# nikhilTkur/Multigrid_Nikhil_C-

Measured on AMD Instinct MI355X. Metric: fine_grid_stencil_updates_per_sec, higher is better.
Workload: dtype f64

## Files before the change

multigrid_nikhil_c-_amd/csrc/mgx_kernels.hpp:

```cpp
#pragma once

#include <hip/hip_runtime.h>
#include "mgx_geom.hpp"
#include <stdint.h>
#include <type_traits>

namespace mgx {

template <int B, int E, typename F> __device__ __forceinline__ void static_for(F&& f)
{
    if constexpr (B < E) {
        f(std::integral_constant<int, B>{});
        static_for<B + 1, E>(f);
    }
}

constexpr int kWave = 64;
constexpr int kBlock = 256;
constexpr int kWavesPerBlock = kBlock / kWave;
constexpr int kOutLanes = kWave - 2;

template <typename T> struct VecOf;
template <> struct VecOf<double> { using type = double2; static constexpr int W = 2; };
template <> struct VecOf<float>  { using type = float4;  static constexpr int W = 4; };
// ... 638 lines not shown
    double a0 = 0.0, a1 = 0.0, a2 = 0.0, a3 = 0.0;
    int i = threadIdx.x;
    for (; i + 3 * kReduceThreads < n; i += 4 * kReduceThreads) {
        a0 += partial[i];
        a1 += partial[i + kReduceThreads];
        a2 += partial[i + 2 * kReduceThreads];
        a3 += partial[i + 3 * kReduceThreads];
    }
    for (; i < n; i += kReduceThreads) a0 += partial[i];
    double acc = (a0 + a1) + (a2 + a3);
    for (int off = 32; off > 0; off >>= 1) acc += __shfl_down(acc, off, kWave);
    if ((threadIdx.x & 63) == 0) wsum[threadIdx.x >> 6] = acc;
    __syncthreads();
    if (threadIdx.x == 0) {
        double s = 0.0;
        for (int w = 0; w < kReduceThreads / kWave; ++w) s += wsum[w];
        out[0] = s;
    }
}

template <typename T> struct Trip { T l, c, r; };

template <typename T, bool FUSED>
__global__ void __launch_bounds__(kBlock)
k_restrict(const T* __restrict__ vin, const T* __restrict__ rhs, T* __restrict__ coarse, T* __restrict__ coarse_zero,
           int N, long pitch, long cpitch, int crow_lo, int crow_hi, int fine_row_off,
           int R, int strips, int chunks, T wgt)
{
    using V = typename VecOf<T>::type;
    constexpr int W = VecOf<T>::W;
    constexpr int CW = W / 2;
    const Tile t = wave_tile(strips, chunks);
    if (!t.active) return;
    const Cols c = lane_cols<W>(t.strip, N, pitch);
    const int I0 = crow_lo + t.chunk * R;
    const int I1 = min(I0 + R, crow_hi);
    const T* pv = vin + c.col;
    const T* pb = rhs + c.col;
    const long ccol = c.col / 2;
    const int NC = N / 2;

    auto row_plain = [&](int y) -> V { V o = vload<V>(pb + (long)y * pitch, c.ld); mask_cols(o, c.col, N); return o; };

    V up, cur, dn;
    int yf = 2 * I0 + fine_row_off - 1;
    if (FUSED) {
        up = vload<V>(pv + (long)(yf - 1) * pitch, c.ld);
        cur = vload<V>(pv + (long)yf * pitch, c.ld);
    }
    auto next_field = [&](int y) -> V {
        if (FUSED) {
            dn = vload<V>(pv + (long)(y + 1) * pitch, c.ld);
            const V bb = vload<V>(pb + (long)y * pitch, c.ld);
            V o = residual_vec(up, cur, dn, bb);
            mask_cols(o, c.col, N);
            up = cur; cur = dn;
            return o;
        } else {
            return row_plain(y);
        }
    };
    auto trips = [&](const V& f, Trip<T>* tr) {
        const T l = from_left(last(f));
        if constexpr (W == 2) { tr[0] = {l, f.x, f.y}; }
        else { tr[0] = {l, f.x, f.y}; tr[1] = {f.y, f.z, f.w}; }
    };

    Trip<T> top[CW], mid[CW], bot[CW];
    { const V f = next_field(yf); trips(f, top); }
    for (int I = I0; I < I1; ++I) {
        const int y = 2 * I + fine_row_off;
        { const V f = next_field(y); trips(f, mid); }
        { const V f = next_field(y + 1); trips(f, bot); }
        T o[CW];
#pragma unroll
        for (int k = 0; k < CW; ++k) {
            T corners = top[k].l + top[k].r; corners = corners + bot[k].l; corners = corners + bot[k].r;
            T edges = mid[k].l + mid[k].r; edges = edges + top[k].c; edges = edges + bot[k].c;
            o[k] = wgt * ((corners + (T)2 * edges) + (T)4 * mid[k].c);
            if (ccol + k == 0 || ccol + k >= NC) o[k] = (T)0;
        }
        if (c.st) {
            T* pc = coarse + (long)I * cpitch + ccol;
            if constexpr (CW == 1) { pc[0] = o[0]; }
            else { *reinterpret_cast<float2*>(pc) = make_float2((float)o[0], (float)o[1]); }
            if (coarse_zero) {
                T* pz = coarse_zero + (long)I * cpitch + ccol;
                if constexpr (CW == 1) { pz[0] = (T)0; }
                else { *reinterpret_cast<float2*>(pz) = make_float2(0.f, 0.f); }
            }
        }
#pragma unroll
        for (int k = 0; k < CW; ++k) top[k] = bot[k];
    }
}

template <typename T, bool ADD>
__global__ void __launch_bounds__(kBlock)
k_prolong(T* __restrict__ v, const T* __restrict__ coarse, int N, long pitch, long cpitch,
          int row_lo, int row_hi, int fine_row_off, int R, int strips, int chunks)
{
    using V = typename VecOf<T>::type;
    constexpr int W = VecOf<T>::W;
    constexpr int CW = W / 2;
    const Tile t = wave_tile(strips, chunks);
    if (!t.active) return;
    const Cols c = lane_cols<W>(t.strip, N, pitch);
    const int r0 = row_lo + t.chunk * R;
    const int r1 = min(r0 + R, row_hi);
    T* pv = v + c.col;
    const long ccol = c.col / 2;
    const bool cld = c.ld && (ccol + CW < cpitch);

    auto crow = [&](int I, T* e) {
        const T* p = coarse + (long)I * cpitch + ccol;
#pragma unroll
        for (int k = 0; k <= CW; ++k) e[k] = cld ? p[k] : (T)0;
    };
    for (int r = r0; r < r1; ++r) {
        const int y = r - fine_row_off;
        const int I = y >> 1;
        T a[CW + 1], b2[CW + 1];
        crow(I, a);
        V add;
        T o[W];
        if ((y & 1) == 0) {
#pragma unroll
            for (int k = 0; k < CW; ++k) { o[2 * k] = a[k]; o[2 * k + 1] = (T)0.5 * (a[k] + a[k + 1]); }
        } else {
            crow(I + 1, b2);
#pragma unroll
            for (int k = 0; k < CW; ++k) {
                o[2 * k] = (T)0.5 * (a[k] + b2[k]);
                o[2 * k + 1] = (T)0.25 * (((a[k] + b2[k]) + a[k + 1]) + b2[k + 1]);
            }
        }
        if constexpr (W == 2) add = make_double2(o[0], o[1]);
        else add = make_float4(o[0], o[1], o[2], o[3]);
        mask_cols(add, c.col, N);
        if (ADD) {
            const V old = vload<V>(pv + (long)r * pitch, c.st);
            if constexpr (W == 2) { add.x = old.x + add.x; add.y = old.y + add.y; }
            else { add.x = old.x + add.x; add.y = old.y + add.y; add.z = old.z + add.z; add.w = old.w + add.w; }
        }
        vstore<V>(pv + (long)r * pitch, add, c.st);
    }
}

template <int K, int POST> constexpr int cycle_halo_cols() { return K + (POST == 1 ? 2 : (POST == 2 ? 1 : 0)); }
template <int K, int POST, int W> constexpr int cycle_out_lanes() { return kWave - 2 * ((cycle_halo_cols<K, POST>() + W - 1) / W); }

template <typename T, int CW> struct CycleState {
    T ct[CW], tc[CW], em[CW], mc[CW];
    double acc;
};

struct CycleWin {
    int row_first, row_last;
    int crow_first, crow_last;
    int emit_lo, emit_hi;
};

struct CycleArgs {
    long cpitch; int NC;
    int r0, r1, y_end;
    bool zero_in;
    CycleWin win;
};

template <typename T, int CW> struct PreFetch { T a[CW + 1], b[CW + 1]; };

template <typename T, bool EDGE>
__device__ __forceinline__ void
coarse_loads(PreFetch<T, VecOf<T>::W / 2>& pe, int y, const T* __restrict__ coarse_e, long cpitch, long ccol, int N, bool cld,
             const CycleWin& win, const FastOut& fo)
{
    constexpr int CW = VecOf<T>::W / 2;
    const int I = y >> 1;
    if constexpr (!EDGE) {
        const int Ia = min(max(I, win.crow_first), win.crow_last), Ib = min(max(I + 1, win.crow_first), win.crow_last);
        const unsigned srow_a = (unsigned)(Ia - fo.crb) * fo.cpitch_bytes, srow_b = (unsigned)(Ib - fo.crb) * fo.cpitch_bytes;
#pragma unroll
        for (int k = 0; k <= CW; ++k) pe.a[k] = bload1_s((T*)nullptr, fo.ce, fo.clane_off + (unsigned)(k * sizeof(T)), srow_a);
#pragma unroll
        for (int k = 0; k <= CW; ++k) pe.b[k] = bload1_s((T*)nullptr, fo.ce, fo.clane_off + (unsigned)(k * sizeof(T)), srow_b);
    } else {
        const bool cl = cld && y > 0 && y < N && I >= win.crow_first && I + (y & 1) <= win.crow_last;
        const bool cl2 = cl && (y & 1);
        const unsigned at = (unsigned)(I - fo.crb) * fo.cpitch_bytes + fo.clane_off;
#pragma unroll
        for (int k = 0; k <= CW; ++k) pe.a[k] = bload1((T*)nullptr, fo.ce, cl ? at + (unsigned)(k * sizeof(T)) : kOobOffset);
#pragma unroll
        for (int k = 0; k <= CW; ++k) pe.b[k] = bload1((T*)nullptr, fo.ce, cl2 ? at + fo.cpitch_bytes + (unsigned)(k * sizeof(T)) : kOobOffset);
    }
}

template <typename T, bool EDGE, bool ZIN = false>
__device__ __forceinline__ void
cycle_loads(typename VecOf<T>::type& in, typename VecOf<T>::type& bn, int y,
            const T* __restrict__ pv, const T* __restrict__ pb, long pitch, int N, int y_end, bool ld, bool zero_in,
            const CycleWin& win, const FastOut& fo)
{
    using V = typename VecOf<T>::type;
    if constexpr (!EDGE) {
        const int yi = min(y, win.row_last), yb = max(min(y - 1, win.row_last), win.row_first);
        if constexpr (ZIN) in = vzero((V*)nullptr);
        else in = bload_s((V*)nullptr, fo.in, fo.lane_off, (unsigned)(yi - fo.rb) * fo.pitch_bytes);
        bn = bload_s((V*)nullptr, fo.rhs, fo.lane_off, (unsigned)(yb - fo.rb) * fo.pitch_bytes);
    } else {
        const bool in_ok = !zero_in && y >= win.row_first && y <= win.row_last && y < y_end;
        const bool b_ok = (y - 1) > 0 && (y - 1) < N && (y - 1) >= win.row_first && (y - 1) <= win.row_last && y <= y_end;
        in = bload((V*)nullptr, fo.in, (ld && in_ok) ? (unsigned)(y - fo.rb) * fo.pitch_bytes + fo.lane_off : kOobOffset);
        bn = bload((V*)nullptr, fo.rhs, (ld && b_ok) ? (unsigned)(y - 1 - fo.rb) * fo.pitch_bytes + fo.lane_off : kOobOffset);
    }
}

constexpr int kBRing = 12;
template <typename T, int K, int POST, int SM> constexpr bool cycle_b_in_lds() { return (sizeof(T) == 8 && K >= 8) || (sizeof(T) == 4 && K >= 10); }
#ifndef MGX_SKEW
#define MGX_SKEW 0
#endif
#ifndef MGX_RING_AHEAD
#define MGX_RING_AHEAD 1
#endif
#ifndef MGX_PRIO_ALT
#define MGX_PRIO_ALT 0
#endif
template <typename T, int K, int PRE, int POST, int SM, int AR> constexpr int cycle_skew()
{
    if (sizeof(T) == 8 && K == 10 && PRE == 1 && POST == 0 && SM == 0 && AR == 0) return 0;
    if (sizeof(T) == 4 && K == 10 && PRE == 0 && POST == 1 && SM == 0) return 0;
    return (MGX_SKEW != 0 && cycle_b_in_lds<T, K, POST, SM>()) ? K / 2 : 0;
}
constexpr int kRawLds = 6;
#ifndef MGX_RAWQ
#define MGX_RAWQ 1
#endif
template <typename T, int K, int PRE, int POST, int SM, int AR> constexpr bool cycle_rawq();
template <typename T> struct LdsVec;
template <> struct LdsVec<double> { typedef double v __attribute__((ext_vector_type(2))); };
template <> struct LdsVec<float> { typedef float v __attribute__((ext_vector_type(4))); };
template <typename T> using lds_vec_ptr = __attribute__((address_space(3))) typename LdsVec<T>::v*;
__device__ __forceinline__ void ring_put(lds_vec_ptr<double> r, int slot, const double2& v)
{
    LdsVec<double>::v t = {v.x, v.y};
    r[slot * kWave] = t;
}
__device__ __forceinline__ double2 ring_get(lds_vec_ptr<double> r, int slot)
{
    const LdsVec<double>::v t = r[slot * kWave];
    return make_double2(t.x, t.y);
}
__device__ __forceinline__ void ring_put(lds_vec_ptr<float> r, int slot, const float4& v)
{
    LdsVec<float>::v t = {v.x, v.y, v.z, v.w};
    r[slot * kWave] = t;
}
__device__ __forceinline__ float4 ring_get(lds_vec_ptr<float> r, int slot)
{
    const LdsVec<float>::v t = r[slot * kWave];
    return make_float4(t.x, t.y, t.z, t.w);
}
constexpr int ring_slot(int m) { return ((m % kBRing) + kBRing) % kBRing; }
template <typename T, int K, int PRE, int POST, int SM, int AR> constexpr bool cycle_rawq()
{
    if (MGX_RAWQ == 0) return false;
    if (PRE != 0 || sizeof(T) != 8) return false;
    if (POST == 2 && AR == 0 && K == 10) return false;
    return cycle_b_in_lds<T, K, POST, SM>() && SM == 0 && POST != 0 && K > kRawLds && cycle_skew<T, K, PRE, POST, SM, AR>() == 0;
}
#ifndef MGX_PFD_DEEP
#define MGX_PFD_DEEP 0
#endif
template <bool BL, int POST, bool EDGE = false> constexpr int cycle_pfd()
{
    if (BL && !EDGE && MGX_PFD_DEEP > 0) return MGX_PFD_DEEP;
    return (BL && (POST == 1 || EDGE)) ? 2 : kPrefetch;
}
constexpr int kPrefetchMax = MGX_PFD_DEEP > kPrefetch ? MGX_PFD_DEEP : kPrefetch;
template <typename T, bool BL, bool EDGE, int POST> constexpr int cycle_cpfd() { return (BL && !(EDGE && POST == 0)) ? cycle_pfd<BL, POST, EDGE>() : 1; }

template <typename T, int K, int PRE, int POST, int SM, bool EDGE, int RP, bool BL, bool ZIN, int AR>
__device__ __forceinline__ void
cycle_step(typename VecOf<T>::type (&lev)[K + 1][3], typename VecOf<T>::type (&bw)[BL ? 1 : K + 1], lds_vec_ptr<T> ring,
           lds_vec_ptr<T> ring2, typename VecOf<T>::type (&rawq)[cycle_rawq<T, K, PRE, POST, SM, AR>() ? kBRing : 1],
           typename VecOf<T>::type (&nin)[kPfStages], typename VecOf<T>::type (&nbn)[kPfStages], PreFetch<T, VecOf<T>::W / 2>& pe,
           CycleState<T, VecOf<T>::W / 2>& cs, int y,
           const T* __restrict__ pv, const T* __restrict__ pb, T* __restrict__ po,
           const T* __restrict__ coarse_e, T* __restrict__ coarse_b, T* __restrict__ coarse_zero, T wgt,
           long pitch, long col, long ccol, int N, const CycleArgs& ca, bool ld, bool cld, bool st, T c0, T c1,
           const FastOut& fo)
{
    using V = typename VecOf<T>::type;
    constexpr int W = VecOf<T>::W;
    constexpr int CW = W / 2;
    constexpr int P = RP % 3;
    constexpr int S_OLD = (P + 1) % 3, S_MID = (P + 2) % 3, S_NEW = P;
    constexpr int bnd_lo = 0;
    const int bnd_hi = N;
    const int r0 = ca.r0, r1 = ca.r1;

    if constexpr (EDGE) __builtin_amdgcn_sched_barrier(0);
    V in = nin[0];
    const V bn = nbn[0];
#pragma unroll
    for (int q = 0; q + 1 < kPfStages; ++q) { nin[q] = nin[q + 1]; nbn[q] = nbn[q + 1]; }
    cycle_loads<T, EDGE, ZIN>(nin[kPfStages - 1], nbn[kPfStages - 1], y + cycle_pfd<BL, POST, EDGE>(), pv, pb, pitch, N, ca.y_end, ld, ca.zero_in, ca.win, fo);
    const ColMask cm = col_mask(col, N);
    if (PRE) {
        T a[CW + 1], b2[CW + 1], o[W];
#pragma unroll
        for (int k = 0; k <= CW; ++k) { a[k] = pe.a[k]; b2[k] = pe.b[k]; }
        coarse_loads<T, EDGE>(pe, y + cycle_cpfd<T, BL, EDGE, POST>(), coarse_e, ca.cpitch, ccol, N, cld, ca.win, fo);
        {
            const bool even = (y & 1) == 0;
#pragma unroll
            for (int k = 0; k < CW; ++k) {
                const T ab = a[k] + b2[k];
                const T ev1 = (T)0.5 * (a[k] + a[k + 1]);
                const T od0 = (T)0.5 * ab;
                const T od1 = (T)0.25 * ((ab + a[k + 1]) + b2[k + 1]);
                o[2 * k] = even ? a[k] : od0;
                o[2 * k + 1] = even ? ev1 : od1;
            }
        }
        V add;
        if constexpr (W == 2) add = make_double2(o[0], o[1]);
        else add = make_float4(o[0], o[1], o[2], o[3]);
        if constexpr (EDGE) mask_sel(add, cm, false);
        if constexpr (W == 2) { in.x = in.x + add.x; in.y = in.y + add.y; }
        else { in.x = in.x + add.x; in.y = in.y + add.y; in.z = in.z + add.z; in.w = in.w + add.w; }
    }
    constexpr bool RAWQ = cycle_rawq<T, K, PRE, POST, SM, AR>();
    constexpr bool PREMUL = (SM == 0 && POST == 0) || RAWQ;
    V b0;
    if constexpr (PREMUL) b0 = vscale(c1, bn);
    else b0 = bn;
    if constexpr (BL) {
        asm volatile("" : "+v"(ring));
        ring_put(ring, ring_slot(RP), b0);
        if constexpr (RAWQ) {
            asm volatile("" : "+v"(ring2));
            rawq[ring_slot(RP)] = ring_get(ring2, RP % kRawLds);
            ring_put(ring2, RP % kRawLds, bn);
        }
    } else {
#pragma unroll
        for (int j = K; j > 0; --j) bw[j] = bw[j - 1];
        bw[0] = b0;
    }
    constexpr int kRingAhead = MGX_RING_AHEAD;
    constexpr int SK = cycle_skew<T, K, PRE, POST, SM, AR>();
    constexpr int SKD = SK > 0 ? 1 : 0;
    constexpr int MLAST = ((POST && !RAWQ) ? K : K - 1) + SKD;
    V rq[BL ? K + 2 : 1];
    auto bwin = [&](auto jc) -> V {
        constexpr int j = decltype(jc)::value;
        if constexpr (j == 0) return b0;
        else if constexpr (BL) return rq[j];
        else return bw[j];
    };
    V dying = lev[SK][S_NEW];
    lev[0][S_NEW] = in;
    auto level = [&](auto jc, auto bc) {
        constexpr int j = decltype(jc)::value;
        constexpr bool inB = decltype(bc)::value;
        const int row = y - j - (inB ? 1 : 0);
        const V cb = bwin(std::integral_constant<int, j - 1 + (inB ? 1 : 0)>{});
        const V& lo = (inB && j == SK + 1) ? dying : lev[j - 1][S_OLD];
        const V& mi = (inB && j == SK + 1) ? lev[j - 1][S_OLD] : lev[j - 1][S_MID];
        const V& hi = (inB && j == SK + 1) ? lev[j - 1][S_MID] : lev[j - 1][S_NEW];
        V o;
        if constexpr (PREMUL) o = jacobi_vec_pre<AR>(lo, mi, hi, cb, c0, c1);
        else o = level_op<T, SM, AR>(j, lo, mi, hi, cb, c0, c1, row + (int)(col & 1));
        if constexpr (EDGE) {
            const int rw = opaque_s(row);
            mask_sel(o, cm, !(rw > bnd_lo && rw < bnd_hi));
        }
        if constexpr (j == K) {
            const unsigned at = (unsigned)(row - fo.rb) * fo.pitch_bytes + fo.lane_off;
            bstore(o, fo.out, (st && row >= r0 && row < r1) ? at : kOobOffset);
        }
        if (j < K || POST) lev[j][S_NEW] = o;
    };
    if constexpr (SK == 0) {
        if constexpr (BL) {
            static_for<1, (kRingAhead < MLAST ? kRingAhead : MLAST) + 1>([&](auto mc) {
                constexpr int m = decltype(mc)::value;
                rq[m] = ring_get(ring, ring_slot(RP - m));
            });
        }
        static_for<1, K + 1>([&](auto jc) {
            constexpr int j = decltype(jc)::value;
            if constexpr (BL && j + kRingAhead <= MLAST) {
                rq[j + kRingAhead] = ring_get(ring, ring_slot(RP - (j + kRingAhead)));
                __builtin_amdgcn_sched_barrier(0);
            }
            level(jc, std::false_type{});
        });
    } else {
        constexpr int NB = K - SK;
        constexpr int NP = SK > NB ? SK : NB;
        rq[SK + 1] = ring_get(ring, ring_slot(RP - (SK + 1)));
        static_for<1, NP + 1>([&](auto ic) {
            constexpr int i = decltype(ic)::value;
            if constexpr (i + 1 <= SK) rq[i] = ring_get(ring, ring_slot(RP - i));
            if constexpr (i + 1 <= NB) rq[SK + i + 1] = ring_get(ring, ring_slot(RP - (SK + i + 1)));
            if constexpr (POST != 0 && i == NP) rq[K + 1] = ring_get(ring, ring_slot(RP - (K + 1)));
            __builtin_amdgcn_sched_barrier(0);
            if constexpr (i <= SK) level(std::integral_constant<int, i>{}, std::false_type{});
            if constexpr (i <= NB) level(std::integral_constant<int, SK + i>{}, std::true_type{});
        });
    }
    if (POST) {
        const int rho = y - K - 1 - SKD;
        V rawb;
        if constexpr (RAWQ) rawb = rawq[ring_slot(RP - (K - kRawLds))];
        else rawb = bwin(std::integral_constant<int, K + SKD>{});
        V res = residual_vec(lev[K][S_OLD], lev[K][S_MID], lev[K][S_NEW], rawb);
        if constexpr (EDGE) {
            const int rw = opaque_s(rho);
            mask_sel(res, cm, !(rw > bnd_lo && rw < bnd_hi));
        }
        if (POST == 2) {
            double r2;
            if constexpr (W == 2) r2 = (double)res.x * (double)res.x + (double)res.y * (double)res.y;
            else r2 = ((double)res.x * (double)res.x + (double)res.y * (double)res.y) +
                      ((double)res.z * (double)res.z + (double)res.w * (double)res.w);
            cs.acc += (st && rho >= r0 && rho < r1) ? r2 : 0.0;
        } else {
            T cl[CW], cc[CW], cr[CW];
            const T l = from_left(last(res));
            if constexpr (W == 2) { cl[0] = l; cc[0] = res.x; cr[0] = res.y; }
            else { cl[0] = l; cc[0] = res.x; cr[0] = res.y; cl[1] = res.y; cc[1] = res.z; cr[1] = res.w; }
            const bool odd = (rho & 1) != 0;
            const int I = (rho - 1) >> 1;
            const bool emit = odd && (2 * I >= r0) && (2 * I < r1) && I >= ca.win.emit_lo && I < ca.win.emit_hi;
            T o[CW];
#pragma unroll
            for (int k = 0; k < CW; ++k) {
                T corners = cs.ct[k] + cl[k]; corners = corners + cr[k];
                const T edges = cs.em[k] + cc[k];
                o[k] = wgt * ((corners + (T)2 * edges) + (T)4 * cs.mc[k]);
                if constexpr (EDGE) o[k] = (ccol + k == 0 || ccol + k >= ca.NC) ? (T)0 : o[k];
            }
            {
                const unsigned at = (st && emit) ? ((unsigned)(I - fo.crb) * fo.cpitch_bytes + fo.clane_off) : kOobOffset;
                if constexpr (CW == 1) { bstore8(o[0], fo.cb, at); bstore8((T)0, fo.cz, at); }
                else { bstore8(make_float2((float)o[0], (float)o[1]), fo.cb, at); bstore8(make_float2(0.f, 0.f), fo.cz, at); }
            }
#pragma unroll
            for (int k = 0; k < CW; ++k) {
                const T lr = cl[k] + cr[k];
                const T em = lr + cs.tc[k];
                cs.em[k] = odd ? cs.em[k] : em;
                cs.mc[k] = odd ? cs.mc[k] : cc[k];
                cs.ct[k] = odd ? lr : cs.ct[k];
                cs.tc[k] = odd ? cc[k] : cs.tc[k];
            }
        }
    }
}

template <typename T, int K, int PRE, int POST, int SM, bool EDGE, bool ZIN, int AR>
__device__ __forceinline__ double
cycle_body(const T* __restrict__ pv, const T* __restrict__ pb, T* __restrict__ po,
           const T* __restrict__ coarse_e, T* __restrict__ coarse_b, T* __restrict__ coarse_zero, T wgt,
           long pitch, long cpitch, long col, int N, int r0, int r1, bool ld, bool st, T c0, T c1, bool zero_in,
           const CycleWin& win, lds_vec_ptr<T> ring, lds_vec_ptr<T> ring2, const FastOut& fo)
{
    constexpr bool BL = cycle_b_in_lds<T, K, POST, SM>();
    constexpr bool RAWQ = cycle_rawq<T, K, PRE, POST, SM, AR>();
    using V = typename VecOf<T>::type;
    constexpr int W = VecOf<T>::W;
    constexpr int CW = W / 2;
    constexpr int ETOP = POST ? 1 : 0;
    constexpr int EBOT = POST == 1 ? 2 : (POST == 2 ? 1 : 0);
    const V Z = vzero((V*)nullptr);
    const long ccol = col / 2;
    const bool cld = ld && (ccol + CW < cpitch);
    V lev[K + 1][3];
    V bw[BL ? 1 : K + 1];
#pragma unroll
    for (int j = 0; j <= K; ++j) { lev[j][0] = Z; lev[j][1] = Z; lev[j][2] = Z; }
#pragma unroll
    for (int j = 0; j < (BL ? 1 : K + 1); ++j) bw[j] = Z;
    if constexpr (BL) {
#pragma unroll
        for (int q = 0; q < kBRing; ++q) ring_put(ring, q, Z);
    }
    V rawq[RAWQ ? kBRing : 1];
#pragma unroll
    for (int q = 0; q < (RAWQ ? kBRing : 1); ++q) rawq[q] = Z;
    if constexpr (RAWQ) {
#pragma unroll
        for (int q = 0; q < kRawLds; ++q) ring_put(ring2, q, Z);
    }
    CycleState<T, CW> cs;
    cs.acc = 0.0;
#pragma unroll
    for (int k = 0; k < CW; ++k) cs.ct[k] = cs.tc[k] = cs.em[k] = cs.mc[k] = (T)0;
    CycleArgs ca;
    ca.cpitch = cpitch; ca.NC = N / 2; ca.r0 = r0; ca.r1 = r1; ca.zero_in = zero_in; ca.win = win;
    const int y0 = r0 - K - ETOP;
    ca.y_end = r1 + K + EBOT + (cycle_skew<T, K, PRE, POST, SM, AR>() > 0 ? 1 : 0);
    constexpr int kRound = BL ? kBRing : trip_steps<T>();
    const int steps = (ca.y_end - y0 + kRound - 1) / kRound * kRound;
    constexpr int PFD = cycle_pfd<BL, POST, EDGE>();
    V nin[PFD][kPfStages], nbn[PFD][kPfStages];
    constexpr int CPFD = cycle_cpfd<T, BL, EDGE, POST>();
    PreFetch<T, CW> pe[CPFD];
#pragma unroll
    for (int q = 0; q < CPFD; ++q) {
#pragma unroll
        for (int k = 0; k <= CW; ++k) { pe[q].a[k] = (T)0; pe[q].b[k] = (T)0; }
    }
#pragma unroll
    for (int q = 0; q < PFD; ++q)
        cycle_loads<T, EDGE, ZIN>(nin[q][0], nbn[q][0], y0 + q, pv, pb, pitch, N, ca.y_end, ld, ca.zero_in, ca.win, fo);
    if (PRE) {
#pragma unroll
        for (int q = 0; q < CPFD; ++q) coarse_loads<T, EDGE>(pe[q], y0 + q, coarse_e, cpitch, ccol, N, cld, ca.win, fo);
    }
#define MGX_CSTEP(RP, Y) cycle_step<T, K, PRE, POST, SM, EDGE, RP, BL, ZIN, AR>(lev, bw, ring, ring2, rawq, nin[(RP) % PFD], nbn[(RP) % PFD], pe[(RP) % CPFD], cs, Y, pv, pb, po, coarse_e, coarse_b, coarse_zero, wgt, pitch, col, ccol, N, ca, ld, cld, st, c0, c1, fo)
    if constexpr (BL) {
#define MGX_CTRIP(Y) do { MGX_CSTEP(0, Y); MGX_CSTEP(1, Y + 1); MGX_CSTEP(2, Y + 2); MGX_CSTEP(3, Y + 3); MGX_CSTEP(4, Y + 4); \
                          MGX_CSTEP(5, Y + 5); MGX_CSTEP(6, Y + 6); MGX_CSTEP(7, Y + 7); MGX_CSTEP(8, Y + 8); MGX_CSTEP(9, Y + 9); \
                          MGX_CSTEP(10, Y + 10); MGX_CSTEP(11, Y + 11); } while (0)
#if MGX_PRIO_ALT
        unsigned hw_id;
        asm volatile("s_getreg_b32 %0, hwreg(HW_REG_HW_ID)" : "=s"(hw_id));
        int turn = (int)(hw_id & 1u);
        for (int y = y0; y < y0 + steps; y += kBRing) {
            if (turn & 1) __builtin_amdgcn_s_setprio(1); else __builtin_amdgcn_s_setprio(0);
            turn ^= 1;
            MGX_CTRIP(y);
        }
        __builtin_amdgcn_s_setprio(0);
#else
        for (int y = y0; y < y0 + steps; y += kBRing) MGX_CTRIP(y);
#endif
#undef MGX_CTRIP
    } else if constexpr (trip_steps<T>() == 12) {
        for (int y = y0; y < y0 + steps; y += 12) {
            MGX_CSTEP(0, y); MGX_CSTEP(1, y + 1); MGX_CSTEP(2, y + 2);
            MGX_CSTEP(3, y + 3); MGX_CSTEP(4, y + 4); MGX_CSTEP(5, y + 5);
            MGX_CSTEP(6, y + 6); MGX_CSTEP(7, y + 7); MGX_CSTEP(8, y + 8);
            MGX_CSTEP(9, y + 9); MGX_CSTEP(10, y + 10); MGX_CSTEP(11, y + 11);
        }
    } else {
        for (int y = y0; y < y0 + steps; y += 3) {
            MGX_CSTEP(0, y); MGX_CSTEP(1, y + 1); MGX_CSTEP(2, y + 2);
        }
    }
#undef MGX_CSTEP
    return cs.acc;
}

template <typename T, int K, int PRE, int POST, int SM, int AR> constexpr int cycle_waves()
{
    return cycle_b_in_lds<T, K, POST, SM>() ? 2 : 1;
}
template <typename T, int K, int PRE, int POST, int SM = 0, int AR = 0>
__global__ void __launch_bounds__(kBlock, (cycle_waves<T, K, PRE, POST, SM, AR>()))
k_jacobi_cycle(const T* __restrict__ vin, const T* __restrict__ rhs, T* __restrict__ vout,
               const T* __restrict__ coarse_e,
               T* __restrict__ coarse_b, T* __restrict__ coarse_zero, T wgt,
               double* __restrict__ partial,
               int N, long pitch, long cpitch, int row_lo, int row_hi, int R, int strips, int chunks, int Re, int chunks_e,
               int row_last0, int Rl, int RB, int n_tall, int n_short, int Rf, T c0, T c1, int zero_in, CycleWin win)
{
    constexpr int W = VecOf<T>::W;
    constexpr int XC = cycle_halo_cols<K, POST>();
    constexpr int HL = (XC + W - 1) / W;
    constexpr int OUT = kWave - 2 * HL;
    constexpr int ETOP = POST ? 1 : 0;
    constexpr int EBOT = POST == 1 ? 2 : (POST == 2 ? 1 : 0);
    __shared__ double wsum[kWavesPerBlock];
    constexpr bool BL = cycle_b_in_lds<T, K, POST, SM>();
    __shared__ typename LdsVec<T>::v bring[BL ? kWavesPerBlock * kBRing * kWave : 1];
    constexpr bool RAWQ = cycle_rawq<T, K, PRE, POST, SM, AR>();
    __shared__ typename LdsVec<T>::v braw[RAWQ ? kWavesPerBlock * kRawLds * kWave : 1];
    const CTile t = cycle_tile(strips, chunks, chunks_e, R, Re, row_lo, row_hi, row_last0, Rl, RB, n_tall, n_short, Rf);
    double acc = 0.0;
#ifdef MGX_WAVE_TRACE
    const long long trace_t0 = wall_clock64();
#endif
    if (t.active) {
        const int lane = threadIdx.x & 63;
        const int wv = __builtin_amdgcn_readfirstlane(threadIdx.x >> 6);
        lds_vec_ptr<T> ring = (lds_vec_ptr<T>)&bring[BL ? (wv * kBRing * kWave + lane) : 0];
        lds_vec_ptr<T> ring2 = (lds_vec_ptr<T>)&braw[RAWQ ? (wv * kRawLds * kWave + lane) : 0];
        const int vx0 = t.strip * OUT - HL;
        const int vx = vx0 + lane;
        const long col = (long)vx * W;
        const bool ld = (vx >= 0) && (col + W <= pitch);
        const bool st = (lane >= HL) && (lane < kWave - HL) && (vx < N / W);
        const int r0 = t.r0, r1 = t.r1;
        constexpr int kRound = BL ? kBRing : trip_steps<T>();
        const int y_first = r0 - K - ETOP - 1;
        constexpr int SKD = cycle_skew<T, K, PRE, POST, SM, AR>() > 0 ? 1 : 0;
        const int y_lastp = (r0 - K - ETOP) + ((r1 + K + EBOT + SKD) - (r0 - K - ETOP) + kRound - 1) / kRound * kRound + kPrefetchMax;
        const int y0c = r0 - K - ETOP, y1c = r1 + K + EBOT - 1;
        bool interior = (vx0 >= 1) && ((long)(vx0 + kWave + 1) * W < N) &&
                        (y0c > 0) && (y1c < N) && (y0c >= win.row_first) && (y1c <= win.row_last);
        if (PRE) interior = interior && (y0c >> 1) >= win.crow_first && ((y1c + 1) >> 1) <= win.crow_last;
        interior = interior && !(PRE != 0 && zero_in);
        FastOut fo;
        fo.rb = max(y_first, win.row_first);
        fo.crb = max(y_first >> 1, win.crow_first);
        fo.pitch_bytes = (unsigned)(pitch * (long)sizeof(T));
        fo.cpitch_bytes = (unsigned)(cpitch * (long)sizeof(T));
        const unsigned f_bytes = rsrc_bytes(fo.rb, win.row_last, fo.pitch_bytes);
        const unsigned c_bytes = rsrc_bytes(fo.crb, win.crow_last, fo.cpitch_bytes);
        const long f_at = (long)fo.rb * pitch, c_at = (long)fo.crb * cpitch;
        fo.out = make_rsrc(vout + f_at, f_bytes);
        fo.in = make_rsrc(vin + f_at, f_bytes);
        fo.rhs = make_rsrc(rhs + f_at, f_bytes);
        fo.ce = make_rsrc(PRE ? coarse_e + c_at : nullptr, (PRE && coarse_e) ? c_bytes : 0u);
        fo.cb = make_rsrc((POST == 1 && coarse_b) ? coarse_b + c_at : nullptr, (POST == 1 && coarse_b) ? c_bytes : 0u);
        fo.cz = make_rsrc((POST == 1 && coarse_zero) ? coarse_zero + c_at : nullptr, (POST == 1 && coarse_zero) ? c_bytes : 0u);
        fo.lane_off = (unsigned)(col * (long)sizeof(T));
        fo.clane_off = (unsigned)((col / 2) * (long)sizeof(T));
        if (interior) {
            if (PRE == 0 && zero_in)
                acc = cycle_body<T, K, PRE, POST, SM, false, PRE == 0, AR>(vin + col, rhs + col, vout + col, coarse_e, coarse_b, coarse_zero, wgt,
                                                                      pitch, cpitch, col, N, r0, r1, true, st, c0, c1, true, win, ring, ring2, fo);
            else
                acc = cycle_body<T, K, PRE, POST, SM, false, false, AR>(vin + col, rhs + col, vout + col, coarse_e, coarse_b, coarse_zero, wgt,
                                                                    pitch, cpitch, col, N, r0, r1, true, st, c0, c1, false, win, ring, ring2, fo);
        } else {
            acc = cycle_body<T, K, PRE, POST, SM, true, false, AR>(vin + col, rhs + col, vout + col, coarse_e, coarse_b, coarse_zero, wgt,
                                                        pitch, cpitch, col, N, r0, r1, ld, st, c0, c1, zero_in != 0, win, ring, ring2, fo);
        }
    }
#ifdef MGX_WAVE_TRACE
    if ((threadIdx.x & 63) == 0) {
        const int w = blockIdx.x * kWavesPerBlock + (threadIdx.x >> 6);
        if (w < (1 << 16)) {
            unsigned hw, xcc;
            asm volatile("s_getreg_b32 %0, hwreg(HW_REG_HW_ID)" : "=s"(hw));
            asm volatile("s_getreg_b32 %0, hwreg(HW_REG_XCC_ID)" : "=s"(xcc));
            g_wave_trace[w] = WaveTrace{trace_t0, wall_clock64(), t.active ? t.strip : -1, t.r0, t.r1,
                                        (int)((hw & 0xFFF0FFFFu) | ((xcc & 0xFu) << 16))};
        }
        if (w == 0) g_wave_trace_n = gridDim.x * kWavesPerBlock;
    }
#endif
    if (POST == 2) {
        for (int off = 32; off > 0; off >>= 1) acc += __shfl_down(acc, off, kWave);
        if ((threadIdx.x & 63) == 0) wsum[threadIdx.x >> 6] = acc;
        __syncthreads();
        if (threadIdx.x == 0) {
            double sum = 0.0;
            for (int w = 0; w < kWavesPerBlock; ++w) sum += wsum[w];
            partial[blockIdx.x] = sum;
        }
    }
}

constexpr int kTileBand = 14;
constexpr int kTileSY = kWavesPerBlock * kTileBand;
constexpr int kTileSX = kWave;

template <int POST> constexpr int tile_extra() { return POST == 1 ? 2 : (POST == 2 ? 1 : 0); }

template <typename T, int SM, int PRE, int POST, int AR = 0>
__global__ void __launch_bounds__(kBlock)
k_tile_smooth(const T* __restrict__ vin, const T* __restrict__ rhs, T* __restrict__ vout,
              const T* __restrict__ coarse_e, T* __restrict__ coarse_b, T* __restrict__ coarse_zero, T wgt,
              double* __restrict__ partial, int N, long pitch, long cpitch, int levels, T c0, T c1,
              int tiles_x, int zero_in, int row_lo, int row_hi, CycleWin win)
{
    constexpr int RW = kTileBand;
    __shared__ T edge[2][kWavesPerBlock][2][kWave];
    __shared__ double wsum[kWavesPerBlock];
    const int He = levels + tile_extra<POST>();
    const int TH = kTileSY - 2 * He, TW = kTileSX - 2 * He;
    const int lane = threadIdx.x & 63;
    const int wv = __builtin_amdgcn_readfirstlane(threadIdx.x >> 6);
    const int ty = blockIdx.x / tiles_x, tx = blockIdx.x - ty * tiles_x;
    const int y0 = wv * RW;
    const int gy0 = row_lo + ty * TH - He + y0;
    const int gx = 1 + tx * TW - He + lane;
    const bool colunk = gx > 0 && gx < N;
    const int NC = N / 2;

    T u[RW], b[RW];
    unsigned rowmask = 0;
#pragma unroll
    for (int i = 0; i < RW; ++i) {
        const int gy = gy0 + i;
        const bool rowok = gy > 0 && gy < N && gy >= win.row_first && gy <= win.row_last;
        if (rowok) rowmask |= 1u << i;
        const bool unk = colunk && rowok;
        const long at = (long)gy * pitch + gx;
        u[i] = (unk && !zero_in) ? vin[at] : (T)0;
        b[i] = unk ? rhs[at] : (T)0;
    }
    if (PRE) {
        const bool codd = (gx & 1) != 0;
#pragma unroll
        for (int i = 0; i < RW; ++i) {
            const int gy = gy0 + i;
            const bool rodd = (gy & 1) != 0;
            const bool unk = colunk && ((rowmask >> i) & 1u) && (gy >> 1) >= win.crow_first && (gy >> 1) + (rodd ? 1 : 0) <= win.crow_last;
            const T* e = coarse_e + (long)(gy >> 1) * cpitch + (gx >> 1);
            const T a00 = unk ? e[0] : (T)0;
            const T a01 = (unk && codd) ? e[1] : (T)0;
            const T a10 = (unk && rodd) ? e[cpitch] : (T)0;
            const T a11 = (unk && rodd && codd) ? e[cpitch + 1] : (T)0;
            const T ev = codd ? (T)0.5 * (a00 + a01) : a00;
            const T od = codd ? (T)0.25 * (((a00 + a10) + a01) + a11) : (T)0.5 * (a00 + a10);
            const T add = rodd ? od : ev;
            u[i] = unk ? u[i] + add : u[i];
        }
    }

    int buf = 0;
    auto halo_rows = [&](const T (&a)[RW], T& up, T& dn) {
        edge[buf][wv][0][lane] = a[0];
        edge[buf][wv][1][lane] = a[RW - 1];
        __syncthreads();
        up = wv > 0 ? edge[buf][wv - 1][1][lane] : (T)0;
        dn = wv < kWavesPerBlock - 1 ? edge[buf][wv + 1][0][lane] : (T)0;
        buf ^= 1;
    };
    for (int j = 1; j <= levels; ++j) {
        T up, dn;
        halo_rows(u, up, dn);
        const bool colact = colunk && lane >= j && lane < kTileSX - j;
        const int ilo = max(j - y0, 0), ihi = min(kTileSY - j - y0, RW);
        const unsigned act = ihi > ilo ? (rowmask & (((1u << (ihi - ilo)) - 1u) << ilo)) : 0u;
        T prev = up;
#pragma unroll
        for (int i = 0; i < RW; ++i) {
            const T cur = u[i];
            const T below = (i == RW - 1) ? dn : u[i + 1];
            const T l = from_left(cur), r = from_right(cur);
            const bool rowact = (act >> i) & 1u;
            if (SM == 0) {
                const T o = jac_pt<AR>(c0, cur, c1 * b[i], c1, nbr(prev, l, r, below));
                u[i] = (colact && rowact) ? o : cur;
            } else {
                const T o = (T)0.25 * (b[i] + nbr(prev, l, r, below));
                u[i] = (colact && rowact && ((gy0 + i + gx) & 1) == ((j - 1) & 1)) ? o : cur;
            }
            prev = cur;
        }
    }

    const bool colout = lane >= He && lane < He + TW && gx < N;
#pragma unroll
    for (int i = 0; i < RW; ++i) {
        const int y = y0 + i, gy = gy0 + i;
        if (y >= He && y < He + TH && gy < N && gy >= row_lo && gy < row_hi && colout) vout[(long)gy * pitch + gx] = u[i];
    }

// ... 389 lines not shown
```

Measured before the change: 1077 billion.

## Specialize fused cycle steps on compile-time row parity to halve coarse loads

```diff
diff --git a/multigrid_nikhil_c-_amd/csrc/mgx_kernels.hpp b/multigrid_nikhil_c-_amd/csrc/mgx_kernels.hpp
--- a/multigrid_nikhil_c-_amd/csrc/mgx_kernels.hpp
+++ b/multigrid_nikhil_c-_amd/csrc/mgx_kernels.hpp
@@ -814,6 +814,7 @@
 
 template <typename T, int CW> struct CycleState {
     T ct[CW], tc[CW], em[CW], mc[CW];
+    T ea[CW + 1];
     double acc;
 };
 
@@ -854,6 +855,24 @@
         for (int k = 0; k <= CW; ++k) pe.a[k] = bload1((T*)nullptr, fo.ce, cl ? at + (unsigned)(k * sizeof(T)) : kOobOffset);
 #pragma unroll
         for (int k = 0; k <= CW; ++k) pe.b[k] = bload1((T*)nullptr, fo.ce, cl2 ? at + fo.cpitch_bytes + (unsigned)(k * sizeof(T)) : kOobOffset);
+    }
+}
+
+template <typename T, bool EDGE>
+__device__ __forceinline__ void
+coarse_row(T (&e)[VecOf<T>::W / 2 + 1], int I, bool cld, const CycleWin& win, const FastOut& fo)
+{
+    constexpr int CW = VecOf<T>::W / 2;
+    if constexpr (!EDGE) {
+        const int Ic = min(max(I, win.crow_first), win.crow_last);
+        const unsigned srow = (unsigned)(Ic - fo.crb) * fo.cpitch_bytes;
+#pragma unroll
+        for (int k = 0; k <= CW; ++k) e[k] = bload1_s((T*)nullptr, fo.ce, fo.clane_off + (unsigned)(k * sizeof(T)), srow);
+    } else {
+        const bool ok = cld && I >= win.crow_first && I <= win.crow_last;
+        const unsigned at = (unsigned)(I - fo.crb) * fo.cpitch_bytes + fo.clane_off;
+#pragma unroll
+        for (int k = 0; k <= CW; ++k) e[k] = bload1((T*)nullptr, fo.ce, ok ? at + (unsigned)(k * sizeof(T)) : kOobOffset);
     }
 }
 
@@ -879,6 +898,14 @@
 
 constexpr int kBRing = 12;
 template <typename T, int K, int POST, int SM> constexpr bool cycle_b_in_lds() { return (sizeof(T) == 8 && K >= 8) || (sizeof(T) == 4 && K >= 10); }
+static_assert(kBRing % 2 == 0, "the deep bodies' step parity needs an even trip");
+template <typename T, int K, int POST, int SM> constexpr int cycle_par() { return cycle_b_in_lds<T, K, POST, SM>() ? ((1 + K + (POST ? 1 : 0)) & 1) : -1; }
+template <typename T, int K, int POST, int SM> __device__ __forceinline__ int cycle_y0(int r0)
+{
+    constexpr int PAR = cycle_par<T, K, POST, SM>();
+    const int y0 = r0 - K - (POST ? 1 : 0);
+    return PAR < 0 ? y0 : y0 - ((y0 - PAR) & 1);
+}
 #ifndef MGX_SKEW
 #define MGX_SKEW 0
 #endif
@@ -942,7 +969,7 @@
 constexpr int kPrefetchMax = MGX_PFD_DEEP > kPrefetch ? MGX_PFD_DEEP : kPrefetch;
 template <typename T, bool BL, bool EDGE, int POST> constexpr int cycle_cpfd() { return (BL && !(EDGE && POST == 0)) ? cycle_pfd<BL, POST, EDGE>() : 1; }
 
-template <typename T, int K, int PRE, int POST, int SM, bool EDGE, int RP, bool BL, bool ZIN, int AR>
+template <typename T, int K, int PRE, int POST, int SM, bool EDGE, int RP, bool BL, bool ZIN, int AR, int YP>
 __device__ __forceinline__ void
 cycle_step(typename VecOf<T>::type (&lev)[K + 1][3], typename VecOf<T>::type (&bw)[BL ? 1 : K + 1], lds_vec_ptr<T> ring,
            lds_vec_ptr<T> ring2, typename VecOf<T>::type (&rawq)[cycle_rawq<T, K, PRE, POST, SM, AR>() ? kBRing : 1],
@@ -970,11 +997,13 @@
     cycle_loads<T, EDGE, ZIN>(nin[kPfStages - 1], nbn[kPfStages - 1], y + cycle_pfd<BL, POST, EDGE>(), pv, pb, pitch, N, ca.y_end, ld, ca.zero_in, ca.win, fo);
     const ColMask cm = col_mask(col, N);
     if (PRE) {
-        T a[CW + 1], b2[CW + 1], o[W];
-#pragma unroll
-        for (int k = 0; k <= CW; ++k) { a[k] = pe.a[k]; b2[k] = pe.b[k]; }
-        coarse_loads<T, EDGE>(pe, y + cycle_cpfd<T, BL, EDGE, POST>(), coarse_e, ca.cpitch, ccol, N, cld, ca.win, fo);
-        {
+        T o[W];
+        bool row_zero = false;
+        if constexpr (YP < 0) {
+            T a[CW + 1], b2[CW + 1];
+#pragma unroll
+            for (int k = 0; k <= CW; ++k) { a[k] = pe.a[k]; b2[k] = pe.b[k]; }
+            coarse_loads<T, EDGE>(pe, y + cycle_cpfd<T, BL, EDGE, POST>(), coarse_e, ca.cpitch, ccol, N, cld, ca.win, fo);
             const bool even = (y & 1) == 0;
 #pragma unroll
             for (int k = 0; k < CW; ++k) {
@@ -985,11 +1014,38 @@
                 o[2 * k] = even ? a[k] : od0;
                 o[2 * k + 1] = even ? ev1 : od1;
             }
+        } else {
+            constexpr int CPFD = cycle_cpfd<T, BL, EDGE, POST>();
+            T b2[CW + 1];
+            if constexpr (YP == 1) {
+#pragma unroll
+                for (int k = 0; k <= CW; ++k) b2[k] = pe.b[k];
+            }
+            if constexpr (((YP + CPFD) & 1) == 1) coarse_row<T, EDGE>(pe.b, ((y + CPFD) >> 1) + 1, cld, ca.win, fo);
+#pragma unroll
+            for (int k = 0; k < CW; ++k) {
+                if constexpr (YP == 0) {
+                    o[2 * k] = cs.ea[k];
+                    o[2 * k + 1] = (T)0.5 * (cs.ea[k] + cs.ea[k + 1]);
+                } else {
+                    const T ab = cs.ea[k] + b2[k];
+                    o[2 * k] = (T)0.5 * ab;
+                    o[2 * k + 1] = (T)0.25 * ((ab + cs.ea[k + 1]) + b2[k + 1]);
+                }
+            }
+            if constexpr (YP == 1) {
+#pragma unroll
+                for (int k = 0; k <= CW; ++k) cs.ea[k] = b2[k];
+            }
+            if constexpr (EDGE) {
+                const int I = y >> 1;
+                row_zero = !(y > 0 && y < N && I >= ca.win.crow_first && I + YP <= ca.win.crow_last);
+            }
         }
         V add;
         if constexpr (W == 2) add = make_double2(o[0], o[1]);
         else add = make_float4(o[0], o[1], o[2], o[3]);
-        if constexpr (EDGE) mask_sel(add, cm, false);
+        if constexpr (EDGE) mask_sel(add, cm, row_zero);
         if constexpr (W == 2) { in.x = in.x + add.x; in.y = in.y + add.y; }
         else { in.x = in.x + add.x; in.y = in.y + add.y; in.z = in.z + add.z; in.w = in.w + add.w; }
     }
@@ -1095,30 +1151,53 @@
             const T l = from_left(last(res));
             if constexpr (W == 2) { cl[0] = l; cc[0] = res.x; cr[0] = res.y; }
             else { cl[0] = l; cc[0] = res.x; cr[0] = res.y; cl[1] = res.y; cc[1] = res.z; cr[1] = res.w; }
-            const bool odd = (rho & 1) != 0;
+            constexpr int RHOP = YP < 0 ? -1 : ((YP + K + 1 + SKD) & 1);
             const int I = (rho - 1) >> 1;
-            const bool emit = odd && (2 * I >= r0) && (2 * I < r1) && I >= ca.win.emit_lo && I < ca.win.emit_hi;
-            T o[CW];
-#pragma unroll
-            for (int k = 0; k < CW; ++k) {
-                T corners = cs.ct[k] + cl[k]; corners = corners + cr[k];
-                const T edges = cs.em[k] + cc[k];
-                o[k] = wgt * ((corners + (T)2 * edges) + (T)4 * cs.mc[k]);
-                if constexpr (EDGE) o[k] = (ccol + k == 0 || ccol + k >= ca.NC) ? (T)0 : o[k];
-            }
-            {
-                const unsigned at = (st && emit) ? ((unsigned)(I - fo.crb) * fo.cpitch_bytes + fo.clane_off) : kOobOffset;
-                if constexpr (CW == 1) { bstore8(o[0], fo.cb, at); bstore8((T)0, fo.cz, at); }
-                else { bstore8(make_float2((float)o[0], (float)o[1]), fo.cb, at); bstore8(make_float2(0.f, 0.f), fo.cz, at); }
-            }
-#pragma unroll
-            for (int k = 0; k < CW; ++k) {
-                const T lr = cl[k] + cr[k];
-                const T em = lr + cs.tc[k];
-                cs.em[k] = odd ? cs.em[k] : em;
-                cs.mc[k] = odd ? cs.mc[k] : cc[k];
-                cs.ct[k] = odd ? lr : cs.ct[k];
-                cs.tc[k] = odd ? cc[k] : cs.tc[k];
+            if constexpr (RHOP < 0) {
+                const bool odd = (rho & 1) != 0;
+                const bool emit = odd && (2 * I >= r0) && (2 * I < r1) && I >= ca.win.emit_lo && I < ca.win.emit_hi;
+                T o[CW];
+#pragma unroll
+                for (int k = 0; k < CW; ++k) {
+                    T corners = cs.ct[k] + cl[k]; corners = corners + cr[k];
+                    const T edges = cs.em[k] + cc[k];
+                    o[k] = wgt * ((corners + (T)2 * edges) + (T)4 * cs.mc[k]);
+                    if constexpr (EDGE) o[k] = (ccol + k == 0 || ccol + k >= ca.NC) ? (T)0 : o[k];
+                }
+                {
+                    const unsigned at = (st && emit) ? ((unsigned)(I - fo.crb) * fo.cpitch_bytes + fo.clane_off) : kOobOffset;
+                    if constexpr (CW == 1) { bstore8(o[0], fo.cb, at); bstore8((T)0, fo.cz, at); }
+                    else { bstore8(make_float2((float)o[0], (float)o[1]), fo.cb, at); bstore8(make_float2(0.f, 0.f), fo.cz, at); }
+                }
+#pragma unroll
+                for (int k = 0; k < CW; ++k) {
+                    const T lr = cl[k] + cr[k];
+                    const T em = lr + cs.tc[k];
+                    cs.em[k] = odd ? cs.em[k] : em;
+                    cs.mc[k] = odd ? cs.mc[k] : cc[k];
+                    cs.ct[k] = odd ? lr : cs.ct[k];
+                    cs.tc[k] = odd ? cc[k] : cs.tc[k];
+                }
+            } else if constexpr (RHOP == 1) {
+                auto close_row = [&](bool emit) {
+                    T o[CW];
+#pragma unroll
+                    for (int k = 0; k < CW; ++k) {
+                        T corners = cs.ct[k] + cl[k]; corners = corners + cr[k];
+                        const T edges = cs.em[k] + cc[k];
+                        o[k] = wgt * ((corners + (T)2 * edges) + (T)4 * cs.mc[k]);
+                        if constexpr (EDGE) o[k] = (ccol + k == 0 || ccol + k >= ca.NC) ? (T)0 : o[k];
+                    }
+                    const unsigned at = (st && emit) ? ((unsigned)(I - fo.crb) * fo.cpitch_bytes + fo.clane_off) : kOobOffset;
+                    if constexpr (CW == 1) { bstore8(o[0], fo.cb, at); bstore8((T)0, fo.cz, at); }
+                    else { bstore8(make_float2((float)o[0], (float)o[1]), fo.cb, at); bstore8(make_float2(0.f, 0.f), fo.cz, at); }
+                };
+                close_row((2 * I >= r0) && (2 * I < r1) && I >= ca.win.emit_lo && I < ca.win.emit_hi);
+#pragma unroll
+                for (int k = 0; k < CW; ++k) { cs.ct[k] = cl[k] + cr[k]; cs.tc[k] = cc[k]; }
+            } else {
+#pragma unroll
+                for (int k = 0; k < CW; ++k) { cs.em[k] = (cl[k] + cr[k]) + cs.tc[k]; cs.mc[k] = cc[k]; }
             }
         }
     }
@@ -1136,7 +1215,6 @@
     using V = typename VecOf<T>::type;
     constexpr int W = VecOf<T>::W;
     constexpr int CW = W / 2;
-    constexpr int ETOP = POST ? 1 : 0;
     constexpr int EBOT = POST == 1 ? 2 : (POST == 2 ? 1 : 0);
     const V Z = vzero((V*)nullptr);
     const long ccol = col / 2;
@@ -1162,9 +1240,12 @@
     cs.acc = 0.0;
 #pragma unroll
     for (int k = 0; k < CW; ++k) cs.ct[k] = cs.tc[k] = cs.em[k] = cs.mc[k] = (T)0;
+#pragma unroll
+    for (int k = 0; k <= CW; ++k) cs.ea[k] = (T)0;
     CycleArgs ca;
     ca.cpitch = cpitch; ca.NC = N / 2; ca.r0 = r0; ca.r1 = r1; ca.zero_in = zero_in; ca.win = win;
-    const int y0 = r0 - K - ETOP;
+    constexpr int PAR = cycle_par<T, K, POST, SM>();
+    const int y0 = cycle_y0<T, K, POST, SM>(r0);
     ca.y_end = r1 + K + EBOT + (cycle_skew<T, K, PRE, POST, SM, AR>() > 0 ? 1 : 0);
     constexpr int kRound = BL ? kBRing : trip_steps<T>();
     const int steps = (ca.y_end - y0 + kRound - 1) / kRound * kRound;
@@ -1181,10 +1262,17 @@
     for (int q = 0; q < PFD; ++q)
         cycle_loads<T, EDGE, ZIN>(nin[q][0], nbn[q][0], y0 + q, pv, pb, pitch, N, ca.y_end, ld, ca.zero_in, ca.win, fo);
     if (PRE) {
-#pragma unroll
-        for (int q = 0; q < CPFD; ++q) coarse_loads<T, EDGE>(pe[q], y0 + q, coarse_e, cpitch, ccol, N, cld, ca.win, fo);
-    }
-#define MGX_CSTEP(RP, Y) cycle_step<T, K, PRE, POST, SM, EDGE, RP, BL, ZIN, AR>(lev, bw, ring, ring2, rawq, nin[(RP) % PFD], nbn[(RP) % PFD], pe[(RP) % CPFD], cs, Y, pv, pb, po, coarse_e, coarse_b, coarse_zero, wgt, pitch, col, ccol, N, ca, ld, cld, st, c0, c1, fo)
+        if constexpr (PAR < 0) {
+#pragma unroll
+            for (int q = 0; q < CPFD; ++q) coarse_loads<T, EDGE>(pe[q], y0 + q, coarse_e, cpitch, ccol, N, cld, ca.win, fo);
+        } else {
+            coarse_row<T, EDGE>(cs.ea, y0 >> 1, cld, ca.win, fo);
+#pragma unroll
+            for (int q = 0; q < CPFD; ++q)
+                if (((PAR + q) & 1) == 1) coarse_row<T, EDGE>(pe[q].b, ((y0 + q) >> 1) + 1, cld, ca.win, fo);
+        }
+    }
+#define MGX_CSTEP(RP, Y) cycle_step<T, K, PRE, POST, SM, EDGE, RP, BL, ZIN, AR, (PAR < 0 ? -1 : ((PAR + (RP)) & 1))>(lev, bw, ring, ring2, rawq, nin[(RP) % PFD], nbn[(RP) % PFD], pe[(RP) % CPFD], cs, Y, pv, pb, po, coarse_e, coarse_b, coarse_zero, wgt, pitch, col, ccol, N, ca, ld, cld, st, c0, c1, fo)
     if constexpr (BL) {
 #define MGX_CTRIP(Y) do { MGX_CSTEP(0, Y); MGX_CSTEP(1, Y + 1); MGX_CSTEP(2, Y + 2); MGX_CSTEP(3, Y + 3); MGX_CSTEP(4, Y + 4); \
                           MGX_CSTEP(5, Y + 5); MGX_CSTEP(6, Y + 6); MGX_CSTEP(7, Y + 7); MGX_CSTEP(8, Y + 8); MGX_CSTEP(9, Y + 9); \
@@ -1260,12 +1348,13 @@
         const bool st = (lane >= HL) && (lane < kWave - HL) && (vx < N / W);
         const int r0 = t.r0, r1 = t.r1;
         constexpr int kRound = BL ? kBRing : trip_steps<T>();
-        const int y_first = r0 - K - ETOP - 1;
+        const int y_first = cycle_y0<T, K, POST, SM>(r0) - 1;
         constexpr int SKD = cycle_skew<T, K, PRE, POST, SM, AR>() > 0 ? 1 : 0;
         const int y_lastp = (r0 - K - ETOP) + ((r1 + K + EBOT + SKD) - (r0 - K - ETOP) + kRound - 1) / kRound * kRound + kPrefetchMax;
         const int y0c = r0 - K - ETOP, y1c = r1 + K + EBOT - 1;
         bool interior = (vx0 >= 1) && ((long)(vx0 + kWave + 1) * W < N) &&
                         (y0c > 0) && (y1c < N) && (y0c >= win.row_first) && (y1c <= win.row_last);
+        interior = interior && (y_first + 1 >= win.row_first);
         if (PRE) interior = interior && (y0c >> 1) >= win.crow_first && ((y1c + 1) >> 1) <= win.crow_last;
         interior = interior && !(PRE != 0 && zero_in);
         FastOut fo;
```

After: 1112 billion, median of 6. 1.03x the previous value.
